# PKU-Alignment/SafeVLA

Measured on AMD Instinct MI355X. Metric: env-steps/sec through PPO-Lagrangian update, higher is better.
Workload: dtype bf16

## Files before the change

safevla_amd/asmgen/amdasm.py:

```python
import struct
from dataclasses import dataclass

import numpy as np

LANES = np.arange(64, dtype=np.int64)
BF16_NAN = 0x7FC0


@dataclass(frozen=True)
class Reg:
    kind: str
    idx: int
    n: int = 1

    def __str__(self):
        if self.n == 1:
            return f"{self.kind}{self.idx}"
        return f"{self.kind}[{self.idx}:{self.idx + self.n - 1}]"

    def __post_init__(self):
        assert not (self.kind in ("v", "a") and self.n > 1 and self.idx % 2), f"misaligned register tuple {self.kind}[{self.idx}:{self.idx + self.n - 1}]"

    def sub(self, i, n=1):
        assert 0 <= i and i + n <= self.n, (self, i, n)
# ... 358 lines not shown
        def fn(w):
            if w.scc:
                w.pc = w.emu.prog.labels[label] - 1
        self._add(f"s_cbranch_scc1 {label}", fn, "branch")

    def s_cbranch_scc0(self, label):
        def fn(w):
            if not w.scc:
                w.pc = w.emu.prog.labels[label] - 1
        self._add(f"s_cbranch_scc0 {label}", fn, "branch")

    def s_memtime(self, d):
        def fn(w):
            w.emu.clock = getattr(w.emu, "clock", 0) + 1000

            def land(t=w.emu.clock):
                w.swr(d, t, 0)
                w.swr(d, 0, 1)
            w.lgq.append(land)
            w.smem_out = getattr(w, "smem_out", 0) + 1
        self._add(f"s_memtime {_txt(d)}", fn, "smem")

    def _valu(self, text, fn):
        self._add(text, fn, "valu")

    def _v2(self, name, d, x, y, f):
        self._valu(f"{name} {_txt(d)}, {_txt(x)}, {_txt(y)}", lambda w: w.wr(d, f(w.rd(x).astype(np.uint64), w.rd(y).astype(np.uint64)) & 0xffffffff))

    def _v3(self, name, d, x, y, z, f):
        self._valu(f"{name} {_txt(d)}, {_txt(x)}, {_txt(y)}, {_txt(z)}",
                   lambda w: w.wr(d, f(w.rd(x).astype(np.uint64), w.rd(y).astype(np.uint64), w.rd(z).astype(np.uint64)) & 0xffffffff))

    def v_mov_b32(self, d, x):
        self._valu(f"v_mov_b32 {_txt(d)}, {_txt(x)}", lambda w: w.wr(d, w.rd(x)))

    def v_swap_b32(self, x, y):
        def fn(w):
            a_, b_ = w.rd(x), w.rd(y)
            w.wr(x, b_)
            w.wr(y, a_)
        self._valu(f"v_swap_b32 {_txt(x)}, {_txt(y)}", fn)

    def v_accvgpr_write_b32(self, d, x):
        self._valu(f"v_accvgpr_write_b32 {_txt(d)}, {_txt(x)}", lambda w: w.wr(d, w.rd(x)))

    def v_accvgpr_read_b32(self, d, x):
        self._valu(f"v_accvgpr_read_b32 {_txt(d)}, {_txt(x)}", lambda w: w.wr(d, w.rd(x)))

    def v_add_u32(self, d, x, y):
        self._v2("v_add_u32", d, x, y, lambda p, q: p + q)

    def v_sub_u32(self, d, x, y):
        self._v2("v_sub_u32", d, x, y, lambda p, q: p - q + (1 << 32))

    def v_lshlrev_b32(self, d, sh, x):
        self._v2("v_lshlrev_b32", d, sh, x, lambda p, q: q << (p & 31))

    def v_lshrrev_b32(self, d, sh, x):
        self._v2("v_lshrrev_b32", d, sh, x, lambda p, q: q >> (p & 31))

    def v_and_b32(self, d, x, y):
        self._v2("v_and_b32", d, x, y, lambda p, q: p & q)

    def v_or_b32(self, d, x, y):
        self._v2("v_or_b32", d, x, y, lambda p, q: p | q)

    def v_xor_b32(self, d, x, y):
        self._v2("v_xor_b32", d, x, y, lambda p, q: p ^ q)

    def v_mul_lo_u32(self, d, x, y):
        self._v2("v_mul_lo_u32", d, x, y, lambda p, q: p * q)

    def v_mul_u32_u24(self, d, x, y):
        self._v2("v_mul_u32_u24", d, x, y, lambda p, q: (p & 0xffffff) * (q & 0xffffff))

    def v_mad_u32_u24(self, d, x, y, z):
        self._v3("v_mad_u32_u24", d, x, y, z, lambda p, q, r: (p & 0xffffff) * (q & 0xffffff) + r)

    def v_lshl_add_u32(self, d, x, sh, z):
        self._v3("v_lshl_add_u32", d, x, sh, z, lambda p, q, r: (p << (q & 31)) + r)

    def v_add_lshl_u32(self, d, x, y, sh):
        self._v3("v_add_lshl_u32", d, x, y, sh, lambda p, q, r: ((p + q) & 0xffffffff) << (r & 31))

    def v_lshl_or_b32(self, d, x, sh, z):
        self._v3("v_lshl_or_b32", d, x, sh, z, lambda p, q, r: (p << (q & 31)) | r)

    def v_and_or_b32(self, d, x, y, z):
        self._v3("v_and_or_b32", d, x, y, z, lambda p, q, r: (p & q) | r)

    def v_add3_u32(self, d, x, y, z):
        self._v3("v_add3_u32", d, x, y, z, lambda p, q, r: p + q + r)

    def v_bfe_u32(self, d, x, off, width):
        self._v3("v_bfe_u32", d, x, off, width, lambda p, q, r: (p >> (q & 31)) & ((1 << (r & 31)) - 1))

    def v_mbcnt_lane_id(self, d):
        self._valu(f"v_mbcnt_lo_u32_b32 {_txt(d)}, -1, 0", lambda w: w.wr(d, np.minimum(LANES, 32).astype(np.uint32)))
        self._valu(f"v_mbcnt_hi_u32_b32 {_txt(d)}, -1, {_txt(d)}", lambda w: w.wr(d, LANES.astype(np.uint32)))

    def v_readfirstlane_b32(self, d, x):
        self.s_nop(1)
        self._v_readfirstlane_raw(d, x)
        self.s_nop(4)

    def _v_readfirstlane_raw(self, d, x):
        def fn(w):
            lanes = np.nonzero(w.lanes())[0]
            w.swr(d, int(w.rd(x)[lanes[0] if len(lanes) else 0]))
        self._valu(f"v_readfirstlane_b32 {_txt(d)}, {_txt(x)}", fn)

    def _vf2(self, name, d, x, y, f):
        def fn(w):
            p, q = w.rd(x).view(np.float32), w.rd(y).view(np.float32)
            with np.errstate(all="ignore"):
                w.wr(d, f(p, q).astype(np.float32).view(np.uint32))
        self._valu(f"{name} {_txt(d)}, {_txt(x)}, {_txt(y)}", fn)

    def v_mul_f32(self, d, x, y):
        self._vf2("v_mul_f32", d, x, y, lambda p, q: p * q)

    def v_add_f32(self, d, x, y):
        self._vf2("v_add_f32", d, x, y, lambda p, q: p + q)

    def v_max_f32(self, d, x, y):
        self._vf2("v_max_f32", d, x, y, np.maximum)

    def v_med3_f32(self, d, x, y, z, neg=(0, 0, 0)):
        def tx(o, n):
            return ("-" if n else "") + (_txt(o) if not isinstance(o, float) else repr(o))

        def fn(w):
            vals = []
            for o, n in zip((x, y, z), neg):
                f = w.rd(o).view(np.float32).astype(np.float32)
                vals.append(-f if n else f)
            with np.errstate(all="ignore"):
                st = np.sort(np.stack(vals), axis=0)[1]
            w.wr(d, st.astype(np.float32).view(np.uint32))
        for o in (x, y, z):
            assert not isinstance(o, float) or o in (0.5, -0.5, 1.0, -1.0, 2.0, -2.0, 4.0, -4.0, 0.0), "VOP3 on gfx9 takes inline constants only"
        self._valu(f"v_med3_f32 {_txt(d)}, {tx(x, neg[0])}, {tx(y, neg[1])}, {tx(z, neg[2])}", fn)

    def _pk_f32(self, name, d, srcs, sel, f):
        assert d.n == 2 and all(isinstance(o, Reg) and o.n == 2 for o in srcs), "packed fp32 operands are 64-bit register pairs"
        assert sum(1 for o in srcs if o.kind == "s") <= 1 or len({(o.kind, o.idx) for o in srcs if o.kind == "s"}) == 1, "constant bus: one SGPR pair"
        sel = list(sel) + [(0, 1)] * (len(srcs) - len(sel))
        op_sel, op_sel_hi = [lo for lo, _ in sel], [hi for _, hi in sel]
        mods = ""
        if any(op_sel):
            mods += " op_sel:[" + ",".join(str(b) for b in op_sel) + "]"
        if not all(op_sel_hi):
            mods += " op_sel_hi:[" + ",".join(str(b) for b in op_sel_hi) + "]"

        def fn(w):
            out = []
            for half in (0, 1):
                with np.errstate(all="ignore"):
                    args = [w.rd(o, sl[half]).view(np.float32).astype(np.float64) for o, sl in zip(srcs, sel)]
                    out.append(f(*args).astype(np.float32).view(np.uint32))
            w.wr(d, out[0], 0)
            w.wr(d, out[1], 1)
        self._valu(f"{name} {_txt(d)}, " + ", ".join(_txt(o) for o in srcs) + mods, fn)

    def v_pk_mul_f32(self, d, x, y, sel=()):
        self._pk_f32("v_pk_mul_f32", d, (x, y), sel, lambda p, q: p * q)

    def v_pk_add_f32(self, d, x, y, sel=()):
        self._pk_f32("v_pk_add_f32", d, (x, y), sel, lambda p, q: p + q)

    def v_pk_fma_f32(self, d, x, y, z, sel=()):
        self._pk_f32("v_pk_fma_f32", d, (x, y, z), sel, lambda p, q, r: p * q + r)

    def v_cvt_pk_bf16_f32(self, d, x, y):
        def fn(w):
            lo = f32_to_bf16_rne(w.rd(x).view(np.float32))
            hi = f32_to_bf16_rne(w.rd(y).view(np.float32))
            w.wr(d, lo | (hi << 16))
        self._valu(f"v_cvt_pk_bf16_f32 {_txt(d)}, {_txt(x)}, {_txt(y)}", fn)

    def v_pk_max_i16(self, d, x, y):
        def fn(w):
            p, q = w.rd(x), w.rd(y)
            out = np.zeros(64, dtype=np.uint32)
            for sh in (0, 16):
                pa = ((p >> sh) & 0xffff).astype(np.uint16).view(np.int16)
                qa = ((q >> sh) & 0xffff).astype(np.uint16).view(np.int16)
                out |= np.maximum(pa, qa).view(np.uint16).astype(np.uint32) << sh
            w.wr(d, out)
        self._valu(f"v_pk_max_i16 {_txt(d)}, {_txt(x)}, {_txt(y)}", fn)

    def v_pk_min_i16(self, d, x, y):
        def fn(w):
            p, q = w.rd(x), w.rd(y)
            out = np.zeros(64, dtype=np.uint32)
            for sh in (0, 16):
                pa = ((p >> sh) & 0xffff).astype(np.uint16).view(np.int16)
                qa = ((q >> sh) & 0xffff).astype(np.uint16).view(np.int16)
                out |= np.minimum(pa, qa).view(np.uint16).astype(np.uint32) << sh
            w.wr(d, out)
        self._valu(f"v_pk_min_i16 {_txt(d)}, {_txt(x)}, {_txt(y)}", fn)

    def _pk16(self, name, d, x, y, f, suffix=""):
        def fn(w):
            p, q = w.rd(x), w.rd(y)
            out = np.zeros(64, dtype=np.uint32)
            for sh in (0, 16):
                pa = ((p >> sh) & 0xffff).astype(np.int64)
                qa = ((q >> sh) & 0xffff).astype(np.int64)
                out |= (f(pa, qa) & 0xffff).astype(np.uint32) << sh
            w.wr(d, out)
        self._valu(f"{name} {_txt(d)}, {_txt(x)}, {_txt(y)}{suffix}", fn)

    def v_pk_min_u16(self, d, x, y):
        self._pk16("v_pk_min_u16", d, x, y, np.minimum)

    def v_pk_sub_u16(self, d, x, y, clamp=False):
        if clamp:
            self._pk16("v_pk_sub_u16", d, x, y, lambda p, q: np.maximum(p - q, 0), " clamp")
        else:
            self._pk16("v_pk_sub_u16", d, x, y, lambda p, q: p - q)

    def v_bfe_i32(self, d, x, off, width):
        def fn(w):
            p = w.rd(x).astype(np.int64)
            o, wd = w.rd(off).astype(np.int64) & 31, w.rd(width).astype(np.int64) & 31
            val = (p >> o) & ((1 << wd) - 1)
            sign = (val >> (wd - 1)) & 1
            val = np.where(sign == 1, val - (1 << wd), val)
            w.wr(d, (val & 0xffffffff).astype(np.uint32))
        self._valu(f"v_bfe_i32 {_txt(d)}, {_txt(x)}, {_txt(off)}, {_txt(width)}", fn)

    def v_bfi_b32(self, d, m, x, y):
        self._v3("v_bfi_b32", d, m, x, y, lambda p, q, r: (p & q) | ((p ^ 0xffffffff) & r))

    def v_permlane32_swap(self, x, y):
        self.s_nop(1)

        def fn(w):
            a_, b_ = w.rd(x), w.rd(y)
            na, nb_ = a_.copy(), b_.copy()
            na[32:] = b_[:32]
            nb_[:32] = a_[32:]
            w.wr(x, na, masked=False)
            w.wr(y, nb_, masked=False)
        self._valu(f"v_permlane32_swap_b32 {_txt(x)}, {_txt(y)}", fn)

    def v_dot2c_f32_bf16(self, d, x, y):
        def fn(w):
            w.in_dot = True
            p, q = w.rd(x), w.rd(y)
            acc = w.rd(d).view(np.float32).astype(np.float64)
            w.in_dot = False
            for sh in (0, 16):
                acc = acc + bf16_to_f32(((p >> sh) & 0xffff).astype(np.uint16)).astype(np.float64) * bf16_to_f32(((q >> sh) & 0xffff).astype(np.uint16)).astype(np.float64)
            w.wr(d, acc.astype(np.float32).view(np.uint32))
            w.dotw[d.idx] = w.nstep
        self._valu(f"v_dot2c_f32_bf16 {_txt(d)}, {_txt(x)}, {_txt(y)}", fn)

    def v_cmp_u32(self, op, d, x, y):
        f = {"ge": np.greater_equal, "lt": np.less, "eq": np.equal, "ne": np.not_equal, "gt": np.greater, "le": np.less_equal}[op]

        def fn(w):
            m = f(w.rd(x), w.rd(y)) & w.lanes()
            val = 0
            for i in np.nonzero(m)[0]:
                val |= 1 << int(i)
            w.swr(d, val & 0xffffffff, 0)
            w.swr(d, val >> 32, 1)
        self._valu(f"v_cmp_{op}_u32 {_txt(d)}, {_txt(x)}, {_txt(y)}", fn)

    def v_cndmask_b32(self, d, x, y, m):
        def fn(w):
            val = w.srd(m, 0) | (w.srd(m, 1) << 32)
            bits = np.array([(val >> i) & 1 for i in range(64)], dtype=bool)
            w.wr(d, np.where(bits, w.rd(y), w.rd(x)))
        self._valu(f"v_cndmask_b32 {_txt(d)}, {_txt(x)}, {_txt(y)}, {_txt(m)}", fn)

    def v_mfma_f32_32x32x16_bf16(self, d, sa, sb, c):
        assert d.n == 16 and sa.n == 4 and sb.n == 4

        def fn(w):
            def frag(r):
                m = np.zeros((32, 16), dtype=np.float32)
                for q in range(4):
                    u = w.rd(r, q)
                    for half in range(2):
                        val = bf16_to_f32(((u >> (16 * half)) & 0xffff).astype(np.uint16))
                        e = 2 * q + half
                        for h in range(2):
                            m[:, 8 * h + e] = val[32 * h:32 * h + 32]
                return m
            A_ = frag(sa).astype(np.float64)
            B_ = frag(sb).astype(np.float64)
            P = A_ @ B_.T
            for r in range(16):
                rows = (r & 3) + 8 * (r >> 2) + 4 * (LANES >> 5)
                cols = LANES & 31
                cin = np.zeros(64, dtype=np.float32) if (isinstance(c, int) and c == 0) else w.rd(c, r).view(np.float32)
                with np.errstate(all="ignore"):
                    out = (P[rows, cols] + cin.astype(np.float64)).astype(np.float32)
                w.wr(d, out.view(np.uint32), r, masked=False)
        self._add(f"v_mfma_f32_32x32x16_bf16 {_txt(d)}, {_txt(sa)}, {_txt(sb)}, {_txt(c)}", fn, "mfma")

    def _ds_addr(self, w, addr, off):
        return w.rd(addr).astype(np.int64) + off

    def ds_read(self, d, addr, off=0):
        nb = 4 * d.n
        name = {4: "ds_read_b32", 8: "ds_read_b64", 16: "ds_read_b128"}[nb]
        assert 0 <= off <= 65535

        def fn(w):
            ad = self._ds_addr(w, addr, off)
            lds = w.emu.lds
            if np.any(ad[w.lanes()] % (8 if nb == 8 else nb if nb < 16 else 16)) or np.any(ad[w.lanes()] + nb > lds.size):
                raise EmuError(f"wave {w.wid}: misaligned / out-of-range LDS read: {name} off {off}")
            data = np.stack([lds[np.clip(ad + b, 0, lds.size - 1)] for b in range(nb)], axis=1)
            w.emu.lds_rd_bytes += nb * 64
            w._chk(d, "load-destination write")
            w.mark(d)
            m = w.lanes()

            def land():
                w.unmark(d)
                words = data.reshape(64, d.n, 4).astype(np.uint32)
                for i in range(d.n):
                    val = words[:, i, 0] | (words[:, i, 1] << 8) | (words[:, i, 2] << 16) | (words[:, i, 3] << 24)
                    arr = w.V if d.kind == "v" else w.A
                    arr[d.idx + i][m] = val[m]
            w.lgq.append(land)
            if len(w.lgq) > 15:
                raise EmuError(f"wave {w.wid}: more than 15 LGKM operations outstanding (4-bit counter)")
        self._add(f"{name} {_txt(d)}, {_txt(addr)}" + (f" offset:{off}" if off else ""), fn, "lds")

    def ds_read_b64_tr_b16(self, d, addr, off=0):
        assert d.n == 2 and 0 <= off <= 65535

        def fn(w):
            ad = self._ds_addr(w, addr, off)
            lds = w.emu.lds
            if np.any(ad % 8) or np.any(ad + 8 > lds.size):
                raise EmuError(f"wave {w.wid}: misaligned / out-of-range transposed LDS read")
            raw = np.stack([lds[ad + b] for b in range(8)], axis=1).astype(np.uint32)
            h = (raw[:, 0::2] | (raw[:, 1::2] << 8))
            out = np.zeros((64, 4), dtype=np.uint32)
            for l in range(64):
                g, i = l & ~15, l & 15
                for r in range(4):
                    out[l, r] = h[g + 4 * r + (i >> 2), i & 3]
            w.emu.lds_rd_bytes += 8 * 64
            w._chk(d, "load-destination write")
            w.mark(d)

            def land():
                w.unmark(d)
                arr = w.V if d.kind == "v" else w.A
                arr[d.idx] = out[:, 0] | (out[:, 1] << 16)
                arr[d.idx + 1] = out[:, 2] | (out[:, 3] << 16)
            w.lgq.append(land)
            if len(w.lgq) > 15:
                raise EmuError(f"wave {w.wid}: more than 15 LGKM operations outstanding (4-bit counter)")
        self._add(f"ds_read_b64_tr_b16 {_txt(d)}, {_txt(addr)}" + (f" offset:{off}" if off else ""), fn, "lds")

    def ds_write(self, addr, src, off=0):
        nb = 4 * src.n
        name = {4: "ds_write_b32", 8: "ds_write_b64", 16: "ds_write_b128"}[nb]
        assert 0 <= off <= 65535

        def fn(w):
            ad = self._ds_addr(w, addr, off)
            lds = w.emu.lds
            m = w.lanes()
            if np.any(ad[m] % min(nb, 16 if nb == 16 else nb)) or np.any(ad[m] + nb > lds.size):
                raise EmuError(f"wave {w.wid}: misaligned / out-of-range LDS write")
            for i in range(src.n):
                val = w.rd(src, i)
                for b in range(4):
                    lds[(ad + 4 * i + b)[m]] = ((val >> (8 * b)) & 0xff).astype(np.uint8)[m]
            w.lgq.append(lambda: None)
            if len(w.lgq) > 15:
                raise EmuError(f"wave {w.wid}: more than 15 LGKM operations outstanding (4-bit counter)")
        self._add(f"{name} {_txt(addr)}, {_txt(src)}" + (f" offset:{off}" if off else ""), fn, "lds")

    @staticmethod
    def _buf_addr(w, vaddr, srd, soff, off):
        base = w.srd(srd, 0) | ((w.srd(srd, 1) & 0xffff) << 32)
        nrec = w.srd(srd, 2)
        voff = w.rd(vaddr).astype(np.int64) if vaddr is not None else np.zeros(64, dtype=np.int64)
        so = w.srd(soff) if isinstance(soff, Reg) else soff
        return base + so + voff + off, voff + off, nrec

    def buffer_load(self, d, vaddr, srd, soff, off=0, nt=False):
        nd = d.n
        name = {1: "buffer_load_dword", 2: "buffer_load_dwordx2", 4: "buffer_load_dwordx4"}[nd]
        assert 0 <= off <= 4095

        def fn(w):
            ad, rng, nrec = self._buf_addr(w, vaddr, srd, soff, off)
            m = w.lanes()
            vals = np.zeros((64, nd), dtype=np.uint32)
            for l in np.nonzero(m)[0]:
                if rng[l] + 4 * nd > nrec:
                    continue
                vals[l] = w.emu.mem_read(int(ad[l]), 4 * nd).view(np.uint32)
            w._chk(d, "load-destination write")
            w.mark(d)
            w.emu.vmem_ld_bytes += 4 * nd * int(m.sum())

            def land():
                w.unmark(d)
                arr = w.V if d.kind == "v" else w.A
                for i in range(nd):
                    arr[d.idx + i][m] = vals[m, i]
            w.vmq.append(land)
            w.retire(w.vmq, 63)
        self._add(f"{name} {_txt(d)}, {_txt(vaddr)}, {_txt(srd)}, {_txt(soff)} offen" + (f" offset:{off}" if off else ""), fn, "vmem")

    def buffer_load_lds_x4(self, vaddr, srd, soff):
        def fn(w):
            ad, rng, nrec = self._buf_addr(w, vaddr, srd, soff, 0)
            m = w.lanes()
            dst0 = w.m0
            if dst0 % 16 or dst0 + 1024 > w.emu.lds.size:
                raise EmuError(f"LDS-DMA destination {dst0}")
            data = np.zeros((64, 16), dtype=np.uint8)
            for l in np.nonzero(m)[0]:
                if rng[l] + 16 <= nrec:
                    data[l] = w.emu.mem_read(int(ad[l]), 16)
            lds = w.emu.lds
            pois = np.tile(np.array([BF16_NAN & 0xff, BF16_NAN >> 8], dtype=np.uint8), 8)
            for l in np.nonzero(m)[0]:
                lds[dst0 + 16 * l: dst0 + 16 * l + 16] = pois
            w.emu.vmem_ld_bytes += 16 * int(m.sum())

            def land():
                for l in np.nonzero(m)[0]:
                    lds[dst0 + 16 * l: dst0 + 16 * l + 16] = data[l]
            w.vmq.append(land)
            w.retire(w.vmq, 63)
        self._add(f"buffer_load_dwordx4 {_txt(vaddr)}, {_txt(srd)}, {_txt(soff)} offen lds", fn, "vmem")

    def global_load_lds_x4(self, voff, sbase, mods=""):
        def fn(w):
            base = w.srd(sbase, 0) | (w.srd(sbase, 1) << 32)
            ad = base + w.rd(voff).astype(np.int64)
            m = w.lanes()
            dst0 = w.m0
            if dst0 % 16 or dst0 + 1024 > w.emu.lds.size:
                raise EmuError(f"LDS-DMA destination {dst0}")
            data = np.zeros((64, 16), dtype=np.uint8)
            for l in np.nonzero(m)[0]:
                data[l] = w.emu.mem_read(int(ad[l]), 16)
            lds = w.emu.lds
            pois = np.tile(np.array([BF16_NAN & 0xff, BF16_NAN >> 8], dtype=np.uint8), 8)
            for l in np.nonzero(m)[0]:
                lds[dst0 + 16 * l: dst0 + 16 * l + 16] = pois
            w.emu.vmem_ld_bytes += 16 * int(m.sum())

            def land():
                for l in np.nonzero(m)[0]:
                    lds[dst0 + 16 * l: dst0 + 16 * l + 16] = data[l]
            w.vmq.append(land)
            w.retire(w.vmq, 63)
        self._add(f"global_load_lds_dwordx4 {_txt(voff)}, {_txt(sbase)}" + (f" {mods}" if mods else ""), fn, "vmem")

    def buffer_atomic_add_f32(self, src, vaddr, srd, soff, off=0):
        assert src.n == 1 and 0 <= off <= 4095

        def fn(w):
            ad, rng, nrec = self._buf_addr(w, vaddr, srd, soff, off)
            m = w.lanes()
            vals = w.rd(src).view(np.float32).copy()

            def land():
                for l in np.nonzero(m)[0]:
                    if rng[l] + 4 <= nrec:
                        _atomic_add_f32(w.emu, int(ad[l]), vals[l])
            w.vmq.append(land)
            w.retire(w.vmq, 63)
        self._add(f"buffer_atomic_add_f32 {_txt(src)}, {_txt(vaddr)}, {_txt(srd)}, {_txt(soff)} offen" + (f" offset:{off}" if off else ""), fn, "vmem")

    def buffer_store(self, src, vaddr, srd, soff, off=0, nt=False):
        nd = src.n
        name = {1: "buffer_store_dword", 2: "buffer_store_dwordx2", 4: "buffer_store_dwordx4"}[nd]
        assert 0 <= off <= 4095

        def fn(w):
            ad, rng, nrec = self._buf_addr(w, vaddr, srd, soff, off)
            m = w.lanes()
            vals = np.stack([w.rd(src, i) for i in range(nd)], axis=1)
            w.emu.vmem_st_bytes += 4 * nd * int(m.sum())

            def land():
                for l in np.nonzero(m)[0]:
                    if rng[l] + 4 * nd > nrec:
                        continue
                    w.emu.mem_write(int(ad[l]), vals[l].view(np.uint8))
            w.vmq.append(land)
            w.retire(w.vmq, 63)
        self._add(f"{name} {_txt(src)}, {_txt(vaddr)}, {_txt(srd)}, {_txt(soff)} offen" + (f" offset:{off}" if off else "") + (" nt" if nt else ""), fn, "vmem")


def _atomic_add_f32(emu, addr, val):
    cur = emu.mem_read(addr, 4).view(np.float32)[0]
    emu.mem_write(addr, np.array([np.float32(cur) + np.float32(val)], dtype=np.float32).view(np.uint8))


class Emu:

    def __init__(self, prog, lds_bytes=163840, nwaves=4):
        self.prog = prog
        self.lds = np.zeros(lds_bytes, dtype=np.uint8)
        rs = np.random.RandomState(7)
        self.lds[:] = rs.randint(0, 256, size=lds_bytes)
        self.bufs = []
        self.next_base = 0x7f0000000000
        self.nwaves = nwaves
        self.lds_rd_bytes = 0
        self.vmem_ld_bytes = 0
        self.vmem_st_bytes = 0

    def alloc(self, arr, writable=False):
        b = arr.view(np.uint8).reshape(-1)
        base = self.next_base
        self.bufs.append((base, b, writable))
        self.next_base += (b.size + 0xffff) & ~0xfff
        return base

    def _find(self, addr, n):
        for base, b, wr in self.bufs:
            if base <= addr and addr + n <= base + b.size:
                return b, addr - base, wr
        raise EmuError(f"memory access fault: address 0x{addr:x} (+{n}) is outside every buffer")

    def mem_read(self, addr, n):
        b, o, _ = self._find(addr, n)
        return b[o:o + n].copy()

    def mem_write(self, addr, data):
        b, o, wr = self._find(addr, data.size)
        if not wr:
            raise EmuError(f"write to read-only buffer at 0x{addr:x}")
        b[o:o + data.size] = data

    def run(self, kernarg, wg_id, order=None, max_steps=50_000_000, wg_id_y=0):
        ka = np.frombuffer(bytes(kernarg), dtype=np.uint8).copy()
        kaddr = self.alloc(ka)
        waves = [Wave(i, self) for i in range(self.nwaves)]
        for w in waves:
            w.S[0] = kaddr & 0xffffffff
            w.S[1] = kaddr >> 32
            w.S[2] = wg_id
            w.S[3] = wg_id_y
            w.V[0] = (np.arange(64) + 64 * w.wid).astype(np.uint32)
        order = list(order) if order is not None else list(range(self.nwaves))
        ops = self.prog.ops
        steps = 0
        while not all(w.done for w in waves):
            progressed = False
            for wi in order:
                w = waves[wi]
                while not w.done and not w.at_barrier:
                    op = ops[w.pc]
                    if op.fn is not None:
                        w.nstep += 1
                        op.fn(w)
                        w.counts[op.kind] = w.counts.get(op.kind, 0) + 1
                    w.pc += 1
                    steps += 1
                    progressed = True
                    if steps > max_steps:
                        raise EmuError("step limit")
            live = [w for w in waves if not w.done]
            if live and all(w.at_barrier for w in live):
                if len(live) != len(waves):
                    raise EmuError("barrier reached by some waves after others ended")
                for w in live:
                    w.at_barrier = False
                progressed = True
            if not progressed:
                raise EmuError("deadlock")
        return waves
```

safevla_amd/asmgen/tn_os_gen.py:

```python
from .amdasm import M0, a, s, v
from .kernelgen import Kernarg, KernelGen

LDS_BYTES = 131072
SLOT = 32768
KARG = Kernarg("TnOsKarg", [("dY", "ptr"), ("ldy", "i64"), ("X", "ptr"), ("ldx", "i64"), ("dW", "ptr"), ("ldw", "i64"), ("db", "ptr"), ("M", "i32"), ("N", "i32"),
                            ("K", "i32"), ("chunk_rows", "i32"), ("ntile", "i32"), ("ntk", "i32"), ("grid", "i32")])
KARG_BYTES = KARG.nbytes

S_DY, S_LDY, S_X, S_LDX, S_DW, S_LDW, S_DB = s(4, 2), s(6, 2), s(8, 2), s(10, 2), s(12, 2), s(14, 2), s(16, 2)
S_M, S_N, S_K, S_CHUNKROWS, S_NTILE, S_NTK = s(18), s(19), s(20), s(21), s(22), s(23)
S_WID, S_WN, S_WK = s(24), s(25), s(26)
S_TILE, S_CHUNK, S_N0, S_K0, S_KT = s(27), s(28), s(29), s(30), s(31)
S_LDY2, S_LDX2, S_2LDY2, S_2LDX2 = s(32), s(33), s(34), s(35)
S_STEPA, S_STEPB = s(36, 2), s(38, 2)
S_PA, S_PB = s(40, 2), s(42, 2)
S_TA, S_TB = s(44, 2), s(46, 2)
SRD_W, SRD_B = s(48, 4), s(52, 4)
S_LEFT, S_DLEFT = s(56), s(57)
S_M0W = s(58)
S_BTURN, S_DOBIAS = s(59), s(60)
S_LDW4, S_ROW = s(61), s(62)
S_T = [s(64 + i) for i in range(12)]
N_SGPR = 102


def ACC(i, j):
    return a((i * 4 + j) * 16, 16)


def FA(f, u):
    return v(f * 32 + u * 4, 4)


def FB(f, u):
    return v(f * 32 + 16 + u * 4, 4)


V_RA = [[v(64 + h * 4 + u) for u in range(4)] for h in range(2)]
V_RB = [[v(72 + h * 4 + u) for u in range(4)] for h in range(2)]
V_SA, V_SB = [v(80), v(81)], [v(82), v(83)]
V_BG = [v(84 + u) for u in range(4)]
V_ONES, V_OFF, V_LANE = v(88), v(89), v(90)
V_T = [v(96 + i) for i in range(16)]


class TnOsGen(KernelGen):
    KARG, LDS_BYTES, N_SGPR = KARG, LDS_BYTES, N_SGPR

    def __init__(self, name="svla_tn_os", dbg=""):
        super().__init__(name, dbg)

    def prologue(self):
        p = self.p
        T = V_T
        p.s_load(s(4, 16), s(0, 2), 0)
        p.s_load(s(20, 4), s(0, 2), 64)
        p.v_and_b32(T[0], 63, v(0))
        p.v_mov_b32(V_LANE, T[0])
        p.v_lshrrev_b32(T[1], 6, v(0))
        p.v_readfirstlane_b32(S_WID, T[1])
        p.s_waitcnt(lgkmcnt=0)
        p.s_lshr_b32(S_WN, S_WID, 1)
        p.s_and_b32(S_WK, S_WID, 1)
        p.s_load(S_T[8], s(0, 2), KARG["grid"])
        p.s_mov_b32(S_T[0], s(2))
        p.s_waitcnt(lgkmcnt=0)
        self.xcd_vid(S_T[6], S_T, S_T[8], "L_XLO", "L_XD")
        self.divmod(S_CHUNK, S_T[6], S_NTILE, "L_DIV", "L_DIVD")
        p.s_mov_b32(S_TILE, S_T[6])
        self.divmod(S_T[7], S_T[6], S_NTK, "L_DIV2", "L_DIV2D")
        p.s_mov_b32(S_KT, S_T[6])
        p.s_lshl_b32(S_N0, S_T[7], 8)
        p.s_lshl_b32(S_K0, S_T[6], 8)
        p.s_mul_i32(S_T[0], S_CHUNK, S_CHUNKROWS)
        p.s_add_u32(S_T[1], S_T[0], S_CHUNKROWS)
        p.s_min_u32(S_T[1], S_T[1], S_M)
        p.s_sub_u32(S_T[1], S_T[1], S_T[0])
        p.s_lshr_b32(S_LEFT, S_T[1], 5)
        p.s_mov_b32(S_DLEFT, S_LEFT)
        p.s_cmp("eq_u32", S_LEFT, 0)
        p.s_cbranch_scc0("L_WORK")
        p.s_endpgm()
        p.label("L_WORK")
        p.s_lshl_b32(S_LDY2, S_LDY.sub(0), 1)
        p.s_lshl_b32(S_LDX2, S_LDX.sub(0), 1)
        p.s_lshl_b32(S_2LDY2, S_LDY2, 1)
        p.s_lshl_b32(S_2LDX2, S_LDX2, 1)
        p.s_lshl_b32(S_LDW4, S_LDW.sub(0), 2)
        for step, ld2 in ((S_STEPA, S_LDY2), (S_STEPB, S_LDX2)):
            p.s_lshl_b32(step.sub(0), ld2, 5)
            p.s_lshr_b32(step.sub(1), ld2, 27)
        p.s_lshl_b32(S_T[2], S_WID, 3)
        p.s_add_u32(S_T[2], S_T[2], S_T[0])
        for ptr, base, ld2, col in ((S_PA, S_DY, S_LDY2, S_N0), (S_PB, S_X, S_LDX2, S_K0)):
            p.s_mul_hi_u32(S_T[4], S_T[2], ld2)
            p.s_mul_i32(S_T[3], S_T[2], ld2)
            p.s_lshl_b32(S_T[5], col, 1)
            p.s_add_u32(S_T[3], S_T[3], S_T[5])
            p.s_addc_u32(S_T[4], S_T[4], 0)
            p.s_add_u32(ptr.sub(0), base.sub(0), S_T[3])
            p.s_addc_u32(ptr.sub(1), base.sub(1), S_T[4])
        p.s_lshl_b32(S_M0W, S_WID, 12)
        p.v_and_b32(T[2], 31, T[0])
        p.v_lshrrev_b32(T[3], 5, T[0])
        p.v_lshrrev_b32(T[4], 2, T[2])
        p.v_and_b32(T[5], 3, T[2])
        for par in range(2):
            p.v_add_u32(T[6], 2 * par, T[3])
            p.v_xor_b32(T[6], T[6], T[4])
            p.v_lshl_add_u32(T[6], T[6], 2, T[5])
            p.v_lshlrev_b32(T[6], 4, T[6])
            p.v_mul_lo_u32(T[7], T[3], S_LDY2)
            p.v_add_u32(V_SA[par], T[6], T[7])
            p.v_mul_lo_u32(T[7], T[3], S_LDX2)
            p.v_add_u32(V_SB[par], T[6], T[7])
        p.v_and_b32(T[2], 15, T[0])
        p.v_lshrrev_b32(T[3], 4, T[0])
        p.v_lshrrev_b32(T[4], 2, T[2])
        p.v_lshrrev_b32(T[5], 1, T[3])
        p.v_lshl_add_u32(T[6], T[5], 3, T[4])
        p.v_lshlrev_b32(T[6], 9, T[6])
        p.v_and_b32(T[7], 1, T[3])
        p.v_lshlrev_b32(T[7], 5, T[7])
        p.v_and_b32(T[8], 3, T[2])
        p.v_lshl_add_u32(T[7], T[8], 3, T[7])
        p.v_add_u32(T[6], T[6], T[7])
        for part, regs, wsel in ((0, V_RA, S_WN), (16384, V_RB, S_WK)):
            p.s_lshl_b32(S_T[2], wsel, 2)
            for u in range(4):
                p.s_add_u32(S_T[3], S_T[2], u)
                p.v_xor_b32(T[9], S_T[3], T[4])
                p.v_lshl_add_u32(T[9], T[9], 6, T[6])
                p.v_add_u32(regs[0][u], part, T[9])
                p.v_add_u32(regs[1][u], part + 2 * SLOT, T[9])
        p.v_mov_b32(V_ONES, 0x3f803f80)
        for u in range(4):
            p.v_mov_b32(V_BG[u], 0)
        for i in range(4):
            for j in range(4):
                for r in range(16):
                    p.v_accvgpr_write_b32(ACC(i, j).sub(r), 0)
        p.s_mov_b32(S_BTURN, S_KT)
        for x, part in ((0, 0), (0, 1), (1, 0), (1, 1), (2, 0), (2, 1), (3, 0)):
            for grp in self.dma_groups(x, part):
                for th in grp:
                    th()
        self.wait_for(vm_tags=[f"dma{0}_{part}_{t}" for part in range(2) for t in range(4)])
        p.s_barrier()
        for u in range(4):
            self.tread(0, 0, 0, "a", u)
            self.tread(0, 0, 0, "b", u)

    def dma_groups(self, x, part):
        p = self.p
        run, cur, two, src = (S_TA, S_PA, S_2LDY2, V_SA) if part == 0 else (S_TB, S_PB, S_2LDX2, V_SB)
        step = S_STEPA if part == 0 else S_STEPB
        groups = []
        for t in range(4):
            def g(t=t):
                if t == 0:
                    p.s_mov_b32(run.sub(0), cur.sub(0))
                    p.s_mov_b32(run.sub(1), cur.sub(1))
                else:
                    p.s_add_u32(run.sub(0), run.sub(0), two)
                    p.s_addc_u32(run.sub(1), run.sub(1), 0)
                p.s_add_u32(M0, S_M0W, (x % 4) * SLOT + part * 16384 + t * 1024)
                p.s_nop(0)
                if "nodma" not in self.dbg:
                    p.global_load_lds_x4(src[t & 1], run)
                    self.vm.issue(f"dma{x % 4}_{part}_{t}")
                if t == 3:
                    if part == 1:
                        p.s_cmp("gt_u32", S_DLEFT, 1)
                        p.s_cselect_b32(S_T[8], S_STEPA.sub(0), 0)
                        p.s_cselect_b32(S_T[9], S_STEPA.sub(1), 0)
                        p.s_cselect_b32(S_T[10], S_STEPB.sub(0), 0)
                        p.s_cselect_b32(S_T[11], S_STEPB.sub(1), 0)
                        p.s_cselect_b32(S_T[7], 1, 0)
                        p.s_sub_u32(S_DLEFT, S_DLEFT, S_T[7])
                        p.s_add_u32(S_PA.sub(0), S_PA.sub(0), S_T[8])
                        p.s_addc_u32(S_PA.sub(1), S_PA.sub(1), S_T[9])
                        p.s_add_u32(S_PB.sub(0), S_PB.sub(0), S_T[10])
                        p.s_addc_u32(S_PB.sub(1), S_PB.sub(1), S_T[11])
            groups.append([g])
        return groups

    def tread(self, f, x, st, which, u):
        pos = x % 4
        regs = (V_RA if which == "a" else V_RB)[pos >> 1][u]
        frag = (FA if which == "a" else FB)(f, u)
        off = (pos & 1) * SLOT + st * 8192
        for hi in range(2):
            self.lg_issue(f"f{f}_{which}{u}", self.p.ds_read_b64_tr_b16, frag.sub(2 * hi, 2), regs, off + hi * 2048)

    def kstep(self, x, st, last_of_slot_barrier):
        p = self.p
        f = st
        fillers = []
        nx, nst = (x, 1) if st == 0 else (x + 1, 0)
        for u in range(4):
            fillers.append(lambda u=u: self.tread(f ^ 1, nx, nst, "a", u))
            fillers.append(lambda u=u: self.tread(f ^ 1, nx, nst, "b", u))
        dpos, dpart = (x + 3, 1) if st == 0 else (x + 4, 0)
        dma = [th for grp in self.dma_groups(dpos, dpart) for th in grp]
        if last_of_slot_barrier:
            nv = self.vm.need({f"dma{(x + 1) % 4}_{part}_{t}" for part in range(2) for t in range(4)})
            self.wait_all(vm=nv if nv is not None else 0)
            p.s_barrier()
        g = 0
        for i in range(4):
            for j in range(4):
                tags = [f"f{f}_a{i}", f"f{f}_b{j}"]
                self.wait_for(lg_tags=tags)
                p.v_mfma_f32_32x32x16_bf16(ACC(i, j), FA(f, i), FB(f, j), ACC(i, j))
                if g < len(fillers) * 2 and g % 2 == 0:
                    fillers[g // 2]()
                if g % 4 == 1 and dma:
                    dma.pop(0)()
                g += 1
        skip = self.uniq("L_NB")
        p.s_cmp("eq_u32", S_DOBIAS, 0)
        p.s_cbranch_scc1(skip)
        for u in range(4):
            for d in range(4):
                p.v_dot2c_f32_bf16(V_BG[u], FA(f, u).sub(d), V_ONES)
        p.label(skip)

    def slot(self, x):
        p = self.p
        p.s_cmp("eq_u32", S_BTURN, 0)
        p.s_cselect_b32(S_DOBIAS, s(3), 0)
        p.s_add_u32(S_BTURN, S_BTURN, 1)
        p.s_cmp("ge_u32", S_BTURN, S_NTK)
        p.s_cselect_b32(S_BTURN, 0, S_BTURN)
        self.kstep(x, 0, False)
        self.kstep(x, 1, True)
        p.s_sub_u32(S_LEFT, S_LEFT, 1)
        p.s_cmp("eq_u32", S_LEFT, 0)
        p.s_cbranch_scc1("L_EPI")

    def build(self):
        p = self.p
        self.prologue()
        p.s_or_b32(S_T[0], S_DB.sub(0), S_DB.sub(1))
        p.s_cmp("lg_u32", S_T[0], 0)
        p.s_cselect_b32(s(3), 1, 0)
        p.s_cmp("eq_u32", S_WK, 0)
        p.s_cselect_b32(s(3), s(3), 0)
        self.scratch(*[lambda x=x: self.slot(x) for x in range(4)])
        p.label("L_LOOP")
        for x in range(4):
            self.slot(x)
        p.s_branch("L_LOOP")
        p.label("L_EPI")
        self.wait_all()
        self.epilogue()
        p.s_endpgm()
        return self

    def epilogue(self):
        p = self.p
        T = V_T
        p.s_lshl_b32(S_T[0], S_WN, 7)
        p.s_add_u32(S_T[0], S_T[0], S_N0)
        p.s_mul_hi_u32(S_T[2], S_T[0], S_LDW4)
        p.s_mul_i32(S_T[1], S_T[0], S_LDW4)
        p.s_lshl_b32(S_T[3], S_WK, 7)
        p.s_add_u32(S_T[3], S_T[3], S_K0)
        p.s_lshl_b32(S_T[3], S_T[3], 2)
        p.s_add_u32(S_T[1], S_T[1], S_T[3])
        p.s_addc_u32(S_T[2], S_T[2], 0)
        p.s_add_u32(SRD_W.sub(0), S_DW.sub(0), S_T[1])
        p.s_addc_u32(S_T[2], S_DW.sub(1), S_T[2])
        p.s_and_b32(SRD_W.sub(1), S_T[2], 0xffff)
        p.s_mov_b32(SRD_W.sub(2), 0xffffffff)
        p.s_mov_b32(SRD_W.sub(3), 0x00020000)
        p.v_and_b32(T[1], 31, V_LANE)
        p.v_lshrrev_b32(T[2], 5, V_LANE)
        p.v_lshlrev_b32(T[2], 2, T[2])
        p.v_mul_lo_u32(T[2], T[2], S_LDW4)
        p.v_lshl_add_u32(V_OFF, T[1], 2, T[2])
        for i in range(4):
            for r in range(16):
                row = 32 * i + (r & 3) + 8 * (r >> 2)
                p.s_mul_i32(S_ROW, S_LDW4, row)
                for j in range(4):
                    p.buffer_atomic_add_f32(ACC(i, j).sub(r), V_OFF, SRD_W, S_ROW, 128 * j)
        done = self.uniq("L_BD")
        p.s_cmp("eq_u32", s(3), 0)
        p.s_cbranch_scc1(done)
        p.s_lshl_b32(S_T[0], S_WN, 7)
        p.s_add_u32(S_T[0], S_T[0], S_N0)
        p.s_lshl_b32(S_T[0], S_T[0], 2)
        p.s_add_u32(SRD_B.sub(0), S_DB.sub(0), S_T[0])
        p.s_addc_u32(S_T[1], S_DB.sub(1), 0)
        p.s_and_b32(SRD_B.sub(1), S_T[1], 0xffff)
        p.s_mov_b32(SRD_B.sub(2), 0xffffffff)
        p.s_mov_b32(SRD_B.sub(3), 0x00020000)
        p.v_lshlrev_b32(T[3], 2, T[1])
        for u in range(4):
            p.buffer_atomic_add_f32(V_BG[u], T[3], SRD_B, 0, 128 * u)
        p.label(done)
        p.s_waitcnt(vmcnt=0)


def generate(dbg=""):
    return TnOsGen(dbg=dbg).build()
```

Baseline: 8180.

## Switch TN outer-product weight-gradient kernel to 16x16x32 MFMA tiling by default

Adds an emulated v_mfma_f32_16x16x32_bf16 instruction and a new code path in the TN weight-gradient kernel that tiles each wave's 128x128 output as 8x8 16x16 MFMA blocks instead of 4x4 32x32 blocks. It uses transposed LDS reads (ds_read_b64_tr_b16), new register maps and swizzles, and an epilogue that atomically adds 16x16 fragments. DMA issue is split into finer pieces interleaved between MFMAs, and the B fragment is double-buffered across slots. The new shape becomes the default, with an environment variable to fall back to 32x32. The cost is a larger VGPR footprint (registers up to about v199) and more atomic and LDS instructions, which may hurt occupancy or the overlap between loads and MFMAs.

Result: no change. 8252 (median of 6 runs) (+0.9%).

```diff
diff --git a/safevla_amd/asmgen/amdasm.py b/safevla_amd/asmgen/amdasm.py
--- a/safevla_amd/asmgen/amdasm.py
+++ b/safevla_amd/asmgen/amdasm.py
@@ -684,6 +684,32 @@
                     out = (P[rows, cols] + cin.astype(np.float64)).astype(np.float32)
                 w.wr(d, out.view(np.uint32), r, masked=False)
         self._add(f"v_mfma_f32_32x32x16_bf16 {_txt(d)}, {_txt(sa)}, {_txt(sb)}, {_txt(c)}", fn, "mfma")
+
+    def v_mfma_f32_16x16x32_bf16(self, d, sa, sb, c):
+        assert d.n == 4 and sa.n == 4 and sb.n == 4
+
+        def fn(w):
+            def frag(r):
+                m = np.zeros((16, 32), dtype=np.float32)
+                for q in range(4):
+                    u = w.rd(r, q)
+                    for half in range(2):
+                        val = bf16_to_f32(((u >> (16 * half)) & 0xffff).astype(np.uint16))
+                        e = 2 * q + half
+                        for h in range(4):
+                            m[:, 8 * h + e] = val[16 * h:16 * h + 16]
+                return m
+            A_ = frag(sa).astype(np.float64)
+            B_ = frag(sb).astype(np.float64)
+            P = A_ @ B_.T
+            for r in range(4):
+                rows = 4 * (LANES >> 4) + r
+                cols = LANES & 15
+                cin = np.zeros(64, dtype=np.float32) if (isinstance(c, int) and c == 0) else w.rd(c, r).view(np.float32)
+                with np.errstate(all="ignore"):
+                    out = (P[rows, cols] + cin.astype(np.float64)).astype(np.float32)
+                w.wr(d, out.view(np.uint32), r, masked=False)
+        self._add(f"v_mfma_f32_16x16x32_bf16 {_txt(d)}, {_txt(sa)}, {_txt(sb)}, {_txt(c)}", fn, "mfma")
 
     def _ds_addr(self, w, addr, off):
         return w.rd(addr).astype(np.int64) + off
diff --git a/safevla_amd/asmgen/tn_os_gen.py b/safevla_amd/asmgen/tn_os_gen.py
--- a/safevla_amd/asmgen/tn_os_gen.py
+++ b/safevla_amd/asmgen/tn_os_gen.py
@@ -1,3 +1,5 @@
+import os
+
 from .amdasm import M0, a, s, v
 from .kernelgen import Kernarg, KernelGen
 
@@ -44,19 +46,44 @@
 V_T = [v(96 + i) for i in range(16)]
 
 
+def ACC16(i, j):
+    return a((i * 8 + j) * 4, 4)
+
+
+def FB16(f, u):
+    return v(f * 32 + u * 4, 4)
+
+
+def FA16(u):
+    return v(64 + u * 4, 4)
+
+
+V16_RA = [[v(128 + h * 8 + u) for u in range(8)] for h in range(2)]
+V16_RB = [[v(144 + h * 8 + u) for u in range(8)] for h in range(2)]
+V16_SA, V16_SB = [v(160 + t) for t in range(4)], [v(164 + t) for t in range(4)]
+V16_BG = [v(168 + u) for u in range(8)]
+V16_ONES, V16_OFF, V16_LANE = v(176), v(177), v(178)
+V16_T = [v(184 + i) for i in range(16)]
+MFMA_SHAPES = ("16x16x32", "32x32x16")
+
+
 class TnOsGen(KernelGen):
     KARG, LDS_BYTES, N_SGPR = KARG, LDS_BYTES, N_SGPR
 
-    def __init__(self, name="svla_tn_os", dbg=""):
+    def __init__(self, name="svla_tn_os", dbg="", mfma="16x16x32"):
         super().__init__(name, dbg)
+        assert mfma in MFMA_SHAPES, mfma
+        self.m16 = mfma == "16x16x32"
+        self.T, self.V_LANE = (V16_T, V16_LANE) if self.m16 else (V_T, V_LANE)
+        self.V_SA, self.V_SB = (V16_SA, V16_SB) if self.m16 else (V_SA, V_SB)
 
     def prologue(self):
         p = self.p
-        T = V_T
+        T = self.T
         p.s_load(s(4, 16), s(0, 2), 0)
         p.s_load(s(20, 4), s(0, 2), 64)
         p.v_and_b32(T[0], 63, v(0))
-        p.v_mov_b32(V_LANE, T[0])
+        p.v_mov_b32(self.V_LANE, T[0])
         p.v_lshrrev_b32(T[1], 6, v(0))
         p.v_readfirstlane_b32(S_WID, T[1])
         p.s_waitcnt(lgkmcnt=0)
@@ -101,6 +128,24 @@
             p.s_add_u32(ptr.sub(0), base.sub(0), S_T[3])
             p.s_addc_u32(ptr.sub(1), base.sub(1), S_T[4])
         p.s_lshl_b32(S_M0W, S_WID, 12)
+        (self.lane_constants16 if self.m16 else self.lane_constants32)()
+        p.s_mov_b32(S_BTURN, S_KT)
+        for x, part in ((0, 0), (0, 1), (1, 0), (1, 1), (2, 0), (2, 1), (3, 0)):
+            for grp in self.dma_groups(x, part):
+                for th in grp:
+                    th()
+        self.wait_for(vm_tags=[f"dma{0}_{part}_{t}" for part in range(2) for t in range(4)])
+        p.s_barrier()
+        if self.m16:
+            for th in self.first_reads16(0):
+                th()
+        else:
+            for u in range(4):
+                self.tread(0, 0, 0, "a", u)
+                self.tread(0, 0, 0, "b", u)
+
+    def lane_constants32(self):
+        p, T = self.p, self.T
         p.v_and_b32(T[2], 31, T[0])
         p.v_lshrrev_b32(T[3], 5, T[0])
         p.v_lshrrev_b32(T[4], 2, T[2])
@@ -140,50 +185,99 @@
             for j in range(4):
                 for r in range(16):
                     p.v_accvgpr_write_b32(ACC(i, j).sub(r), 0)
-        p.s_mov_b32(S_BTURN, S_KT)
-        for x, part in ((0, 0), (0, 1), (1, 0), (1, 1), (2, 0), (2, 1), (3, 0)):
-            for grp in self.dma_groups(x, part):
-                for th in grp:
-                    th()
-        self.wait_for(vm_tags=[f"dma{0}_{part}_{t}" for part in range(2) for t in range(4)])
-        p.s_barrier()
-        for u in range(4):
-            self.tread(0, 0, 0, "a", u)
-            self.tread(0, 0, 0, "b", u)
-
-    def dma_groups(self, x, part):
-        p = self.p
-        run, cur, two, src = (S_TA, S_PA, S_2LDY2, V_SA) if part == 0 else (S_TB, S_PB, S_2LDX2, V_SB)
-        step = S_STEPA if part == 0 else S_STEPB
-        groups = []
+
+    def lane_constants16(self):
+        p, T = self.p, self.T
+        p.v_and_b32(T[2], 31, T[0])
+        p.v_lshrrev_b32(T[3], 5, T[0])
+        p.v_lshlrev_b32(T[4], 2, T[3])
+        p.v_xor_b32(T[4], T[4], T[2])
+        p.v_mul_lo_u32(T[5], T[3], S_LDY2)
+        p.v_mul_lo_u32(T[6], T[3], S_LDX2)
         for t in range(4):
-            def g(t=t):
+            p.v_xor_b32(T[7], 8 * (t & 1) + 2 * (t >> 1), T[4])
+            p.v_lshl_add_u32(V16_SA[t], T[7], 4, T[5])
+            p.v_lshl_add_u32(V16_SB[t], T[7], 4, T[6])
+        p.v_and_b32(T[2], 15, T[0])
+        p.v_lshrrev_b32(T[3], 4, T[0])
+        p.v_lshrrev_b32(T[4], 2, T[2])
+        p.v_and_b32(T[5], 1, T[3])
+        p.v_lshrrev_b32(T[6], 1, T[3])
+        p.v_lshlrev_b32(T[6], 4, T[6])
+        p.v_lshl_add_u32(T[6], T[5], 2, T[6])
+        p.v_add_u32(T[6], T[6], T[4])
+        p.v_lshlrev_b32(T[6], 9, T[6])
+        p.v_and_b32(T[7], 1, T[2])
+        p.v_lshl_add_u32(T[6], T[7], 3, T[6])
+        p.v_lshlrev_b32(T[8], 2, T[4])
+        p.v_lshl_add_u32(T[8], T[5], 1, T[8])
+        p.v_lshrrev_b32(T[7], 1, T[2])
+        p.v_and_b32(T[7], 1, T[7])
+        p.v_or_b32(T[8], T[8], T[7])
+        for part, regs, wsel in ((0, V16_RA, S_WN), (16384, V16_RB, S_WK)):
+            p.s_lshl_b32(S_T[2], wsel, 4)
+            for u in range(8):
+                p.s_add_u32(S_T[3], S_T[2], 2 * u)
+                p.v_xor_b32(T[9], S_T[3], T[8])
+                p.v_lshl_add_u32(T[9], T[9], 4, T[6])
+                p.v_add_u32(regs[0][u], part, T[9])
+                p.v_add_u32(regs[1][u], part + 2 * SLOT, T[9])
+        p.v_mov_b32(V16_ONES, 0x3f803f80)
+        for u in range(8):
+            p.v_mov_b32(V16_BG[u], 0)
+        for r in range(256):
+            p.v_accvgpr_write_b32(a(r), 0)
+
+    def dma_pieces(self, x, part):
+        p = self.p
+        run, cur, two, src = (S_TA, S_PA, S_2LDY2, self.V_SA) if part == 0 else (S_TB, S_PB, S_2LDX2, self.V_SB)
+        pieces = []
+        for t in range(4):
+            def step(t=t):
                 if t == 0:
                     p.s_mov_b32(run.sub(0), cur.sub(0))
                     p.s_mov_b32(run.sub(1), cur.sub(1))
                 else:
                     p.s_add_u32(run.sub(0), run.sub(0), two)
                     p.s_addc_u32(run.sub(1), run.sub(1), 0)
+
+            def issue(t=t):
                 p.s_add_u32(M0, S_M0W, (x % 4) * SLOT + part * 16384 + t * 1024)
                 p.s_nop(0)
                 if "nodma" not in self.dbg:
-                    p.global_load_lds_x4(src[t & 1], run)
+                    p.global_load_lds_x4(src[t % len(src)], run)
                     self.vm.issue(f"dma{x % 4}_{part}_{t}")
-                if t == 3:
-                    if part == 1:
-                        p.s_cmp("gt_u32", S_DLEFT, 1)
-                        p.s_cselect_b32(S_T[8], S_STEPA.sub(0), 0)
-                        p.s_cselect_b32(S_T[9], S_STEPA.sub(1), 0)
-                        p.s_cselect_b32(S_T[10], S_STEPB.sub(0), 0)
-                        p.s_cselect_b32(S_T[11], S_STEPB.sub(1), 0)
-                        p.s_cselect_b32(S_T[7], 1, 0)
-                        p.s_sub_u32(S_DLEFT, S_DLEFT, S_T[7])
-                        p.s_add_u32(S_PA.sub(0), S_PA.sub(0), S_T[8])
-                        p.s_addc_u32(S_PA.sub(1), S_PA.sub(1), S_T[9])
-                        p.s_add_u32(S_PB.sub(0), S_PB.sub(0), S_T[10])
-                        p.s_addc_u32(S_PB.sub(1), S_PB.sub(1), S_T[11])
-            groups.append([g])
-        return groups
+            after = []
+            if t == 3 and part == 1:
+                def sel0():
+                    p.s_cmp("gt_u32", S_DLEFT, 1)
+                    p.s_cselect_b32(S_T[8], S_STEPA.sub(0), 0)
+                    p.s_cselect_b32(S_T[9], S_STEPA.sub(1), 0)
+
+                def sel1():
+                    p.s_cselect_b32(S_T[10], S_STEPB.sub(0), 0)
+                    p.s_cselect_b32(S_T[11], S_STEPB.sub(1), 0)
+                    p.s_cselect_b32(S_T[7], 1, 0)
+
+                def adv_a():
+                    p.s_sub_u32(S_DLEFT, S_DLEFT, S_T[7])
+                    p.s_add_u32(S_PA.sub(0), S_PA.sub(0), S_T[8])
+                    p.s_addc_u32(S_PA.sub(1), S_PA.sub(1), S_T[9])
+
+                def adv_b():
+                    p.s_add_u32(S_PB.sub(0), S_PB.sub(0), S_T[10])
+                    p.s_addc_u32(S_PB.sub(1), S_PB.sub(1), S_T[11])
+                after = [sel0, sel1, adv_a, adv_b]
+            pieces.append((step, issue, after))
+        return pieces
+
+    def dma_groups(self, x, part):
+        def run_all(step, issue, after):
+            step()
+            issue()
+            for th in after:
+                th()
+        return [[lambda pc=pc: run_all(*pc)] for pc in self.dma_pieces(x, part)]
 
     def tread(self, f, x, st, which, u):
         pos = x % 4
@@ -226,6 +320,51 @@
                 p.v_dot2c_f32_bf16(V_BG[u], FA(f, u).sub(d), V_ONES)
         p.label(skip)
 
+    def tread16(self, which, u, x, hi):
+        pos = x % 4
+        regs = (V16_RA if which == "a" else V16_RB)[pos >> 1][u]
+        frag, tag = (FA16(u), f"y{u}") if which == "a" else (FB16(x & 1, u), f"x{x & 1}_{u}")
+        self.lg_issue(tag, self.p.ds_read_b64_tr_b16, frag.sub(2 * hi, 2), regs, (pos & 1) * SLOT + hi * 4096)
+
+    def first_reads16(self, x):
+        frags = [("a", 0)] + [("b", u) for u in range(8)] + [("a", 1)]
+        return [lambda w=w, u=u, hi=hi: self.tread16(w, u, x, hi) for w, u in frags for hi in range(2)]
+
+    def half16(self, x, h):
+        p = self.p
+        if h == 0:
+            reads = [lambda u=u, hi=hi: self.tread16("a", u, x, hi) for u in range(2, 8) for hi in range(2)]
+            dpos, dpart = x + 3, 1
+        else:
+            nv = self.vm.need({f"dma{(x + 1) % 4}_{part}_{t}" for part in range(2) for t in range(4)})
+            self.wait_all(vm=nv if nv is not None else 0)
+            p.s_barrier()
+            reads = self.first_reads16(x + 1)
+            dpos, dpart = x + 4, 0
+        gaps = [[r] for r in reads] + [[] for _ in range(32 - len(reads))]
+        g = len(reads)
+        for step, issue, after in self.dma_pieces(dpos, dpart):
+            gaps[g].append(step)
+            gaps[g + 1].append(issue)
+            for n, th in enumerate(after):
+                gaps[g + 2 + n].append(th)
+            g += 3 if len(reads) > 16 else 4
+        g = 0
+        for i in range(4 * h, 4 * h + 4):
+            for j in range(8):
+                self.wait_for(lg_tags=[f"y{i}", f"x{x & 1}_{j}"])
+                p.v_mfma_f32_16x16x32_bf16(ACC16(i, j), FA16(i), FB16(x & 1, j), ACC16(i, j))
+                for th in gaps[g]:
+                    th()
+                g += 1
+        skip = self.uniq("L_NB")
+        p.s_cmp("eq_u32", S_DOBIAS, 0)
+        p.s_cbranch_scc1(skip)
+        for u in range(4 * h, 4 * h + 4):
+            for d in range(4):
+                p.v_dot2c_f32_bf16(V16_BG[u], FA16(u).sub(d), V16_ONES)
+        p.label(skip)
+
     def slot(self, x):
         p = self.p
         p.s_cmp("eq_u32", S_BTURN, 0)
@@ -233,8 +372,12 @@
         p.s_add_u32(S_BTURN, S_BTURN, 1)
         p.s_cmp("ge_u32", S_BTURN, S_NTK)
         p.s_cselect_b32(S_BTURN, 0, S_BTURN)
-        self.kstep(x, 0, False)
-        self.kstep(x, 1, True)
+        if self.m16:
+            self.half16(x, 0)
+            self.half16(x, 1)
+        else:
+            self.kstep(x, 0, False)
+            self.kstep(x, 1, True)
         p.s_sub_u32(S_LEFT, S_LEFT, 1)
         p.s_cmp("eq_u32", S_LEFT, 0)
         p.s_cbranch_scc1("L_EPI")
@@ -260,7 +403,7 @@
 
     def epilogue(self):
         p = self.p
-        T = V_T
+        T = self.T
         p.s_lshl_b32(S_T[0], S_WN, 7)
         p.s_add_u32(S_T[0], S_T[0], S_N0)
         p.s_mul_hi_u32(S_T[2], S_T[0], S_LDW4)
@@ -275,6 +418,8 @@
         p.s_and_b32(SRD_W.sub(1), S_T[2], 0xffff)
         p.s_mov_b32(SRD_W.sub(2), 0xffffffff)
         p.s_mov_b32(SRD_W.sub(3), 0x00020000)
+        if self.m16:
+            return self.epilogue16()
         p.v_and_b32(T[1], 31, V_LANE)
         p.v_lshrrev_b32(T[2], 5, V_LANE)
         p.v_lshlrev_b32(T[2], 2, T[2])
@@ -289,6 +434,15 @@
         done = self.uniq("L_BD")
         p.s_cmp("eq_u32", s(3), 0)
         p.s_cbranch_scc1(done)
+        self.bias_srd()
+        p.v_lshlrev_b32(T[3], 2, T[1])
+        for u in range(4):
+            p.buffer_atomic_add_f32(V_BG[u], T[3], SRD_B, 0, 128 * u)
+        p.label(done)
+        p.s_waitcnt(vmcnt=0)
+
+    def bias_srd(self):
+        p = self.p
         p.s_lshl_b32(S_T[0], S_WN, 7)
         p.s_add_u32(S_T[0], S_T[0], S_N0)
         p.s_lshl_b32(S_T[0], S_T[0], 2)
@@ -297,12 +451,29 @@
         p.s_and_b32(SRD_B.sub(1), S_T[1], 0xffff)
         p.s_mov_b32(SRD_B.sub(2), 0xffffffff)
         p.s_mov_b32(SRD_B.sub(3), 0x00020000)
+
+    def epilogue16(self):
+        p, T = self.p, self.T
+        p.v_and_b32(T[1], 15, V16_LANE)
+        p.v_lshrrev_b32(T[2], 4, V16_LANE)
+        p.v_lshlrev_b32(T[2], 2, T[2])
+        p.v_mul_lo_u32(T[2], T[2], S_LDW4)
+        p.v_lshl_add_u32(V16_OFF, T[1], 2, T[2])
+        for i in range(8):
+            for r in range(4):
+                p.s_mul_i32(S_ROW, S_LDW4, 16 * i + r)
+                for j in range(8):
+                    p.buffer_atomic_add_f32(ACC16(i, j).sub(r), V16_OFF, SRD_W, S_ROW, 64 * j)
+        done = self.uniq("L_BD")
+        p.s_cmp("eq_u32", s(3), 0)
+        p.s_cbranch_scc1(done)
+        self.bias_srd()
         p.v_lshlrev_b32(T[3], 2, T[1])
-        for u in range(4):
-            p.buffer_atomic_add_f32(V_BG[u], T[3], SRD_B, 0, 128 * u)
+        for u in range(8):
+            p.buffer_atomic_add_f32(V16_BG[u], T[3], SRD_B, 0, 64 * u)
         p.label(done)
         p.s_waitcnt(vmcnt=0)
 
 
-def generate(dbg=""):
-    return TnOsGen(dbg=dbg).build()
+def generate(dbg="", mfma=None):
+    return TnOsGen(dbg=dbg, mfma=mfma or os.environ.get("SVLA_TN_OS_MFMA") or "16x16x32").build()
```
